# hmomin/FinEnvs

Hardware: NVIDIA B200
Metric: env_steps_per_sec (higher is better)
Workload: dtype f32/f64

## Files before the change

finenvs_b200/csrc/fe_step.cu:

```cuda
#include "finenvs_b200.h"
#include "fe_common.cuh"
#include "fe_metrics.cuh"

#include <cuda.h>
#include <cuda_runtime.h>
#include <stdint.h>
#include <stdlib.h>

#include <atomic>
#include <mutex>
#include <vector>

namespace {

constexpr int kThreads = 128;
constexpr int kMaxTileEnvs = kThreads;
constexpr int kSmemHeader = 16;
constexpr int kSmemMax = 226 * 1024;

__device__ __forceinline__ float fmul(float a, float b) { return __fmul_rn(a, b); }
__device__ __forceinline__ float fadd(float a, float b) { return __fadd_rn(a, b); }
__device__ __forceinline__ float fsub(float a, float b) { return __fsub_rn(a, b); }
__device__ __forceinline__ double dmul(double a, double b) { return __dmul_rn(a, b); }
__device__ __forceinline__ double dadd(double a, double b) { return __dadd_rn(a, b); }
// ... 423 lines not shown
    }
    __syncthreads();

    if (warp < kPipeBook) {
        const bool ahead = !kObserve && k.rewards_mirror != nullptr;
        auto tile_env = [&](int t) { return ((int64_t)blockIdx.x + (int64_t)t * gridDim.x) * TE + lane; };
        auto tile_active = [&](int t) { return t < ntiles && lane < TE && tile_env(t) < p.num_envs; };
        EnvLoads ld, ld_next;
        ld.seg = 0; ld.ptr = 0; ld.cash = 0.0f; ld.lng = 0.0f; ld.sht = 0.0f; ld.act = 0.0f; ld.margin = 0.0;
        ld_next = ld;
        if (ahead && tile_active(warp)) ld = env_load_state(st, actions, tile_env(warp));
        for (int t = warp; t < ntiles; t += kPipeBook) {
            const int q = t % kPipeQ;
            if (ahead && tile_active(t + kPipeBook)) ld_next = env_load_state(st, actions, tile_env(t + kPipeBook));
            mbar_wait(desc_free(q), ((t / kPipeQ) & 1) ^ 1);
            const int64_t env0 = ((int64_t)blockIdx.x + (int64_t)t * gridDim.x) * TE;
            const int nvalid = (int)min((int64_t)TE, p.num_envs - env0);
            EnvResult r;
            r.done = 0; r.newly_terminated = 0; r.fin_return = 0.0; r.fin_len = 0; r.row0 = 0; r.posfeat = 0.0;
            const bool active = lane < nvalid;
            if (active) {
                const int64_t i = env0 + lane;
                if (kObserve) r = env_observe(p, s, st, k, i);
                else {
                    if (!ahead) ld = env_load_state(st, actions, i);
                    r = env_compute<OutT>(p, s, st, k, i, ld, env_load_bar(p, s, ld), rewards, dones, stats != nullptr, step);
                }
                d_row0[q * TE + lane] = r.row0;
                reinterpret_cast<OutT *>(d_pf + q * TE)[lane] = (OutT)r.posfeat;
            }
            ld = ld_next;
            if (!kObserve && k.dones_bits_out) {
                const unsigned word = __ballot_sync(0xFFFFFFFFu, active && r.done);
                if (lane == 0) k.dones_bits_out[env0 >> 5] = word;
            }
            if (!kObserve) accumulate_stats(stats, r, active);
            __syncwarp();
            if (lane == 0) mbar_arrive(desc_full(q));
        }
    } else {
        const int mtid = tid - kPipeBook * 32;
        int e_u[RPT], j_u[RPT];
#pragma unroll
        for (int u = 0; u < RPT; ++u) {
            e_u[u] = (mtid + u * kMovers) / W;
            j_u[u] = (mtid + u * kMovers) - e_u[u] * W;
        }
        const Row4<OutT> *series_rows = reinterpret_cast<const Row4<OutT> *>(s.logret);
        auto tile_rows = [&](int t) {
            const int64_t env0 = ((int64_t)blockIdx.x + (int64_t)t * gridDim.x) * TE;
            return (int)min((int64_t)TE, p.num_envs - env0) * W;
        };
        auto gather = [&](int t, Row4<OutT>(&buf)[RPT]) {
            const int q = t % kPipeQ;
            mbar_wait(desc_full(q), (t / kPipeQ) & 1);
            const int nrows = tile_rows(t);
            const uint32_t stage = kPipeSIn > 0 ? smem_u32(in_ring + (t % (kPipeSIn > 0 ? kPipeSIn : 1)) * in_stage) : 0u;
#pragma unroll
            for (int u = 0; u < RPT; ++u) {
                const int r = mtid + u * kMovers;
                if (r < nrows) {
                    const Row4<OutT> *src = series_rows + d_row0[q * TE + e_u[u]] + j_u[u];
                    if constexpr (kPipeSIn == 0) {
                        buf[u] = ldg_row(src);
                    } else {
                        cp_async16(stage + (uint32_t)r * sizeof(Row4<OutT>), src);
                        if constexpr (sizeof(OutT) == 8)
                            cp_async16(stage + (uint32_t)r * sizeof(Row4<OutT>) + 16, reinterpret_cast<const char *>(src) + 16);
                    }
                }
            }
            if constexpr (kPipeSIn > 0) cp_async_arrive_noinc(in_full(t % (kPipeSIn > 0 ? kPipeSIn : 1)));
        };
        Row4<OutT> cur[RPT], nxt[RPT];
        constexpr int kAhead = kPipeSIn > 0 ? kPipeSIn : 1;
        if constexpr (kPipeSIn == 0) {
            if (ntiles > 0) gather(0, cur);
        } else {
            for (int t = 0; t < kAhead && t < ntiles; ++t) gather(t, nxt);
        }
        for (int t = 0; t < ntiles; ++t) {
            const int q = t % kPipeQ, so = t % kPipeSOut;
            const int64_t env0 = ((int64_t)blockIdx.x + (int64_t)t * gridDim.x) * TE;
            const int nrows = tile_rows(t);
            if constexpr (kPipeSIn == 0) {
                if (t + 1 < ntiles) gather(t + 1, nxt);
            } else {
                mbar_wait(in_full(t % kAhead), (t / kAhead) & 1);
                const Row4<OutT> *in_rows = reinterpret_cast<const Row4<OutT> *>(in_ring + (t % kAhead) * in_stage);
#pragma unroll
                for (int u = 0; u < RPT; ++u) {
                    const int r = mtid + u * kMovers;
                    if (r < nrows) cur[u] = in_rows[r];
                }
            }
            if (t >= kPipeSOut) {
                if (mtid == 0) asm volatile("cp.async.bulk.wait_group.read %0;" ::"n"(kPipeSOut - 1) : "memory");
                named_bar_sync(1, kMovers);
            }
            OutT *out_tile = reinterpret_cast<OutT *>(out_ring + so * out_stage);
            const OutT *pf = reinterpret_cast<const OutT *>(d_pf + q * TE);
#pragma unroll
            for (int u = 0; u < RPT; ++u) {
                const int r = mtid + u * kMovers;
                if (r < nrows) {
                    OutT *o = out_tile + (size_t)r * 5;
                    if constexpr (sizeof(OutT) == 4) {
                        o[0] = cur[u].v.x; o[1] = cur[u].v.y; o[2] = cur[u].v.z; o[3] = cur[u].v.w;
                    } else {
                        o[0] = cur[u].a.x; o[1] = cur[u].a.y; o[2] = cur[u].b.x; o[3] = cur[u].b.y;
                    }
                    o[4] = pf[e_u[u]];
                }
            }
            const size_t out_bytes = (size_t)nrows * 5 * sizeof(OutT);
            OutT *dst = obs + (size_t)env0 * W * 5;
            if ((out_bytes & 15) == 0) {
                fence_proxy_async_smem();
                named_bar_sync(1, kMovers);
                if (mtid == 0) {
                    bulk_store_hint(dst, smem_u32(out_tile), (uint32_t)out_bytes, l2_policy_evict_first());
                    bulk_commit();
                }
            } else {
                named_bar_sync(1, kMovers);
                for (int f = mtid; f < nrows * 5; f += kMovers) dst[f] = out_tile[f];
                named_bar_sync(1, kMovers);
            }
            if constexpr (kPipeSIn == 0) {
                if (mtid == 0) mbar_arrive(desc_free(q));
#pragma unroll
                for (int u = 0; u < RPT; ++u) cur[u] = nxt[u];
            } else {
                if (mtid == 0) mbar_arrive(desc_free(q));
                if (t + kAhead < ntiles) gather(t + kAhead, nxt);
            }
        }
        if (mtid == 0) bulk_wait_read_all();
    }
}

#ifndef FE_GATHER_BOOK
#define FE_GATHER_BOOK 6
#endif
#ifndef FE_GATHER_MOVE
#define FE_GATHER_MOVE 12
#endif
#ifndef FE_GATHER_STAGES
#define FE_GATHER_STAGES 3
#endif
#ifndef FE_GATHER_FLUSH_SPINS
#define FE_GATHER_FLUSH_SPINS 2000
#endif
constexpr int kGaBook = FE_GATHER_BOOK;
constexpr int kGaMove = FE_GATHER_MOVE;
constexpr int kGaThreads = (kGaBook + kGaMove) * 32;
constexpr int kGaQ = 32;
constexpr int kGaMaxStages = 4;
constexpr int kGaBarBytes = 1280;
constexpr int kGaPitch = 80;

static_assert((2 * kGaQ + kGaMove * kGaMaxStages) * 8 + 16 <= kGaBarBytes, "mbarrier area too small");
__host__ __device__ inline int ga_row_bytes(bool f64) { return f64 ? 40 : 20; }
__host__ __device__ inline int ga_phase_shift(bool f64) { return f64 ? 1 : 2; }
__host__ __device__ inline int64_t ga_rows_per_phase(int64_t num_rows, int W, bool f64) {
    const int P = 1 << ga_phase_shift(f64);
    return (num_rows + P - 1) / P + (W + P - 1) / P + 8;
}
__host__ __device__ inline size_t ga_table_bytes(int64_t num_rows, int W, bool f64) {
    return (size_t)(1 << ga_phase_shift(f64)) * (size_t)ga_rows_per_phase(num_rows, W, f64) * kGaPitch + 4096;
}
__host__ __device__ inline int ga_parts(int W, bool f64) {
    const int wb = ga_row_bytes(f64) * W;
    if (W <= 0 || (wb % 16) != 0) return 0;
    if (wb <= 2048) return 1;
    if (wb <= 4096 && ((wb / 2) % kGaPitch) == 0 && W <= 128) return 2;
    return 0;
}
__host__ __device__ inline bool ga_window_ok(int W, bool f64) { return ga_parts(W, f64) != 0; }
__host__ __device__ inline uint32_t ga_slot_pitch(int W, bool f64) {
    const int parts = ga_parts(W, f64);
    return ((4u / (uint32_t)(parts ? parts : 1)) * ga_row_bytes(f64) * W + 127u) & ~127u;
}
template <typename OutT> __host__ __device__ inline size_t gather_desc_bytes() {
    return ((size_t)kGaQ * (4 + 32 * (4 + sizeof(OutT))) + 127) & ~(size_t)127;
}
template <typename OutT> __host__ __device__ inline size_t gather_smem_bytes(int W, int S) {
    return kGaBarBytes + gather_desc_bytes<OutT>() + (size_t)kGaMove * S * ga_slot_pitch(W, sizeof(OutT) == 8);
}

__device__ __forceinline__ void tma_gather4(uint32_t dst_smem, const CUtensorMap *map, int r0, int r1, int r2, int r3, uint32_t bar,
                                            uint64_t policy) {
    asm volatile(
        "cp.async.bulk.tensor.2d.shared::cluster.global.tile::gather4.mbarrier::complete_tx::bytes.L2::cache_hint"
        " [%0], [%1, {%2, %3, %4, %5, %6}], [%7], %8;"
        ::"r"(dst_smem), "l"(map), "r"(0), "r"(r0), "r"(r1), "r"(r2), "r"(r3), "r"(bar), "l"(policy)
        : "memory");
}

#ifdef FE_GATHER_CLOCKS
__device__ unsigned long long fe_gather_clk[16];
__device__ unsigned long long fe_gather_block_ns[3 * 160];
__device__ __forceinline__ unsigned long long ga_globaltimer() {
    unsigned long long t;
    asm volatile("mov.u64 %0, %%globaltimer;" : "=l"(t));
    return t;
}
#define GA_CLK(var) const long long var = clock64()
#define GA_ACC(slot, a, b) acc[slot] += (b) - (a)
#else
#define GA_CLK(var)
#define GA_ACC(slot, a, b)
#endif

template <typename OutT, bool kObserve, int kParts>
__global__ void __launch_bounds__(kGaThreads, 1)
fe_gather_kernel(const __grid_constant__ CUtensorMap tmap, const FeParams p, const FeSeries s, const FeState st, const Consts k,
                 const float *__restrict__ actions, OutT *__restrict__ obs, OutT *__restrict__ rewards,
                 int32_t *__restrict__ dones, FeStats *stats, const uint64_t step_arg, const uint64_t *__restrict__ step_dev,
                 const int S, const int rows_per_phase, unsigned int *__restrict__ sched) {
    constexpr bool kF64 = sizeof(OutT) == 8;
    constexpr int kUnitEnvs = 4 / kParts;
    constexpr int kTileUnits = 32 / kUnitEnvs;
    constexpr int kUnitShift = kParts == 1 ? 3 : 4;
    static_assert(kParts == 1 || kParts == 2, "a window is fetched in one or two parts");
    extern __shared__ __align__(128) unsigned char smem[];
    const uint64_t step = step_dev ? *step_dev : step_arg;
    const int W = p.window;
    const int tid = threadIdx.x, warp = tid >> 5, lane = tid & 31;
    const int ntiles_all = (int)((p.num_envs + 31) / 32);
    const uint32_t bars = smem_u32(smem);
    auto desc_full = [&](int q) { return bars + 8u * q; };
    auto desc_free = [&](int q) { return bars + 8u * (kGaQ + q); };
    auto slot_full = [&](int m, int si) { return bars + 8u * (2 * kGaQ + m * kGaMaxStages + si); };
    unsigned int *claim = reinterpret_cast<unsigned int *>(smem + kGaBarBytes - 16);
    int32_t *d_tile = reinterpret_cast<int32_t *>(smem + kGaBarBytes);
    int32_t *d_row = d_tile + kGaQ;
    OutT *d_pf = reinterpret_cast<OutT *>(smem + kGaBarBytes + (size_t)kGaQ * (4 + 32 * 4));
    unsigned char *ring = smem + kGaBarBytes + gather_desc_bytes<OutT>();
    const uint32_t pitch = ga_slot_pitch(W, kF64);

#ifdef FE_GATHER_CLOCKS
    if (tid == 0 && blockIdx.x < 160) {
        unsigned smid;
        asm volatile("mov.u32 %0, %%smid;" : "=r"(smid));
        fe_gather_block_ns[3 * blockIdx.x] = ga_globaltimer();
        fe_gather_block_ns[3 * blockIdx.x + 2] = smid;
        fe_gather_block_ns[3 * blockIdx.x + 1] = 0;
    }
#endif
    if (tid == 0) {
        for (int q = 0; q < kGaQ; ++q) { mbar_init(desc_full(q), 1); mbar_init(desc_free(q), kTileUnits); }
        for (int m = 0; m < kGaMove; ++m)
            for (int si = 0; si < kGaMaxStages; ++si) mbar_init(slot_full(m, si), 1);
        claim[0] = 0; claim[1] = 0;
        mbar_fence_init();
    }
    __syncthreads();

    if (warp < kGaBook) {
        const int shift = ga_phase_shift(kF64);
#ifdef FE_GATHER_CLOCKS
        long long acc[16] = {0};
        int ntl = 0;
#endif
        const bool ahead = !kObserve && k.rewards_mirror != nullptr;
        auto take_claim = [&](int &n, int &t) {
            n = 0; t = 0;
            if (lane == 0) {
                while (atomicCAS(&claim[0], 0u, 1u) != 0u) {}
                n = (int)claim[1];
                claim[1] = (unsigned)n + 1;
                t = (int)atomicAdd(&sched[0], 1u);
                __threadfence_block();
                atomicExch(&claim[0], 0u);
            }
            n = __shfl_sync(0xFFFFFFFFu, n, 0);
            t = __shfl_sync(0xFFFFFFFFu, t, 0);
        };
        auto first_hop = [&](int t, EnvLoads &ld) {
            const int64_t i = (int64_t)t * 32 + lane;
            if (!kObserve && t < ntiles_all && i < p.num_envs) ld = env_load_state(st, actions, i);
        };
        int n, t, n_next = 0, t_next = 0;
        EnvLoads ld, ld_next;
        ld.seg = 0; ld.ptr = 0; ld.cash = 0.0f; ld.lng = 0.0f; ld.sht = 0.0f; ld.act = 0.0f; ld.margin = 0.0;
        ld_next = ld;
        take_claim(n, t);
        first_hop(t, ld);
        for (;;) {
            const int q = n & (kGaQ - 1);
            if (ahead && t < ntiles_all) {
                take_claim(n_next, t_next);
                first_hop(t_next, ld_next);
            }
            GA_CLK(c0);
            if (lane == 0) mbar_wait(desc_free(q), ((n / kGaQ) & 1) ^ 1);
            __syncwarp();
            GA_CLK(c1);
            GA_ACC(8, c0, c1);
            if (t >= ntiles_all) {
                if (lane == 0) { d_tile[q] = -1; mbar_arrive(desc_full(q)); }
                break;
            }
            const int64_t i = (int64_t)t * 32 + lane;
            const bool active = i < p.num_envs;
            EnvResult r;
            r.done = 0; r.newly_terminated = 0; r.fin_return = 0.0; r.fin_len = 0; r.row0 = 0; r.posfeat = 0.0;
            if (active) {
                if (kObserve) r = env_observe(p, s, st, k, i);
                else r = env_compute<OutT>(p, s, st, k, i, ld, env_load_bar(p, s, ld), rewards, dones, stats != nullptr, step);
            }
            d_row[q * 32 + lane] = (int32_t)((r.row0 & ((1 << shift) - 1)) * rows_per_phase + (r.row0 >> shift));
            d_pf[q * 32 + lane] = (OutT)r.posfeat;
            if (lane == 0) d_tile[q] = t;
            if (!kObserve && k.dones_bits_out) {
                const unsigned word = __ballot_sync(0xFFFFFFFFu, active && r.done);
                if (lane == 0) k.dones_bits_out[t] = word;
            }
            if (!kObserve) accumulate_stats(stats, r, active);
            __syncwarp();
            if (lane == 0) mbar_arrive(desc_full(q));
            GA_CLK(c2);
            GA_ACC(9, c1, c2);
#ifdef FE_GATHER_CLOCKS
            ++ntl;
#endif
            if (ahead) { n = n_next; t = t_next; ld = ld_next; }
            else { take_claim(n, t); first_hop(t, ld); }
        }
        if (!kObserve && k.dones_bits_host) {
            if (lane == 0) {
                __threadfence();
                atomicAdd(&sched[2], 1u);
            }
            if (warp == 0) {
                int ok = 1;
                if (lane == 0) {
                    const unsigned want = gridDim.x * (unsigned)kGaBook;
                    int spins = 0;
                    while (ld_acquire_gpu(&sched[2]) < want) {
                        if (++spins > FE_GATHER_FLUSH_SPINS) { ok = 0; break; }
                        __nanosleep(100);
                    }
                    if (!ok) atomicOr(&sched[3], 1u);
                }
                ok = __shfl_sync(0xFFFFFFFFu, ok, 0);
                const int per = (((ntiles_all + (int)gridDim.x - 1) / (int)gridDim.x) + 31) & ~31;
                const int w_begin = (int)blockIdx.x * per;
                const int w_end = !ok ? w_begin : w_begin + per < ntiles_all ? w_begin + per : ntiles_all;
                constexpr int kBatch = 8;
                for (int w0 = w_begin + lane; w0 < w_end; w0 += kBatch * 32) {
                    uint32_t v[kBatch];
#pragma unroll
                    for (int j = 0; j < kBatch; ++j) v[j] = w0 + 32 * j < w_end ? __ldcg(k.dones_bits_out + w0 + 32 * j) : 0u;
#pragma unroll
                    for (int j = 0; j < kBatch; ++j)
                        if (w0 + 32 * j < w_end) k.dones_bits_host[w0 + 32 * j] = v[j];
                }
            }
        }
#ifdef FE_GATHER_CLOCKS
        if (blockIdx.x == 0 && tid == 0) { fe_gather_clk[8] = acc[8]; fe_gather_clk[9] = acc[9]; fe_gather_clk[10] = ntl; }
#endif
    } else {
#ifdef FE_GATHER_CLOCKS
        long long acc[16] = {0};
        const long long mover_t0 = clock64();
#endif
        const int m = warp - kGaBook;
        const uint32_t row_b = (uint32_t)ga_row_bytes(kF64) * W, unit_b = kUnitEnvs * row_b;
        const int part_rows = (int)(row_b / 2) / kGaPitch;
        unsigned char *slots = ring + (size_t)m * S * pitch;
        constexpr int kRounds = (kParts == 1 && kF64) ? 2 : 4;
        uint32_t round_mask = 0;
#pragma unroll
        for (int kk = 0; kk < kRounds; ++kk) round_mask |= (uint32_t)(lane + 32 * kk < W) << kk;
        const uint32_t env_stride = (uint32_t)W * 5;
        const uint64_t keep = l2_policy_evict_last(), stream_out = l2_policy_evict_first();
        static_assert((kGaQ & (kGaQ - 1)) == 0, "kGaQ must be a power of two");
        int iss_u = m, iss_si = 0;
        int issued = 0;
        bool open = true;
        auto issue = [&]() {
            const int n = iss_u >> kUnitShift, g = iss_u & (kTileUnits - 1), q = n & (kGaQ - 1);
            GA_CLK(c0);
            mbar_wait(desc_full(q), (n / kGaQ) & 1);
            GA_CLK(c1);
            GA_ACC(4, c0, c1);
            if (d_tile[q] < 0) { open = false; return; }
            int4 rows4;
            if constexpr (kParts == 1) {
                rows4 = *reinterpret_cast<const int4 *>(d_row + q * 32 + 4 * g);
            } else {
                const int2 r2 = *reinterpret_cast<const int2 *>(d_row + q * 32 + 2 * g);
                rows4 = make_int4(r2.x, r2.x + part_rows, r2.y, r2.y + part_rows);
            }
#ifdef FE_GATHER_NOLOAD
            if (rows4.x == -12345)
#endif
            {
                mbar_arrive_expect_tx(slot_full(m, iss_si), unit_b);
                tma_gather4(smem_u32(slots + (size_t)iss_si * pitch), &tmap, rows4.x, rows4.y, rows4.z, rows4.w, slot_full(m, iss_si),
                            keep);
            }
#ifdef FE_GATHER_NOLOAD
            mbar_arrive(slot_full(m, iss_si));
#endif
            ++issued;
            iss_u += kGaMove;
            iss_si = iss_si + 1 == S ? 0 : iss_si + 1;
            GA_CLK(c2);
            GA_ACC(5, c1, c2);
        };
        if (lane == 0)
            for (int i = 0; i < S && open; ++i) issue();
        int u = m, si = 0;
        uint32_t slot_phase = 0;
        int n_iss = __shfl_sync(0xFFFFFFFFu, issued, 0);
        for (int i = 0; i < n_iss; ++i) {
            const int n = u >> kUnitShift, g = u & (kTileUnits - 1), q = n & (kGaQ - 1);
            GA_CLK(c0);
            if (lane == 0) mbar_wait(slot_full(m, si), (slot_phase >> si) & 1u);
            __syncwarp();
            GA_CLK(c1);
            GA_ACC(0, c0, c1);
            unsigned char *slot = slots + (size_t)si * pitch;
            const OutT *pf = d_pf + q * 32 + kUnitEnvs * g;
            OutT *col = reinterpret_cast<OutT *>(slot) + 5 * lane + 4;
#ifdef FE_GATHER_NOPF
            if (pf[0] == (OutT)12345.678)
#endif
#pragma unroll
            for (int e = 0; e < kUnitEnvs; ++e) {
                const OutT v = pf[e];
#pragma unroll
                for (int kk = 0; kk < kRounds; ++kk)
                    if (round_mask & (1u << kk)) col[e * env_stride + 160 * kk] = v;
            }
            GA_CLK(c1b);
            GA_ACC(1, c1, c1b);
#ifndef FE_GATHER_NOFENCE
            fence_proxy_async_smem();
#endif
            __syncwarp();
            GA_CLK(c2);
            GA_ACC(11, c1b, c2);
            if (lane == 0) {
                const int64_t env0 = (int64_t)d_tile[q] * 32 + kUnitEnvs * g;
                const int64_t left = p.num_envs - env0;
                const int nv = left >= kUnitEnvs ? kUnitEnvs : (left > 0 ? (int)left : 0);
#ifdef FE_GATHER_NOSTORE
                if (nv > 4)
#else
                if (nv > 0)
#endif
                {
                    bulk_store_hint(obs + (size_t)env0 * W * 5, smem_u32(slot), (uint32_t)nv * row_b, stream_out);
                    bulk_commit();
                }
                mbar_arrive(desc_free(q));
                GA_CLK(c3);
                GA_ACC(2, c2, c3);
                if (open) {
                    bulk_wait_read_all();
                    GA_CLK(c4);
                    GA_ACC(3, c3, c4);
                    issue();
                }
            }
            __syncwarp();
            n_iss = __shfl_sync(0xFFFFFFFFu, issued, 0);
            slot_phase ^= 1u << si;
            u += kGaMove;
            si = si + 1 == S ? 0 : si + 1;
        }
        if (lane == 0) bulk_wait_read_all();
#ifdef FE_GATHER_CLOCKS
        if (lane == 0 && blockIdx.x < 160) atomicMax(&fe_gather_block_ns[3 * blockIdx.x + 1], ga_globaltimer());
        if (blockIdx.x == 0 && m == 0 && lane == 0) { for (int c = 0; c < 6; ++c) fe_gather_clk[c] = acc[c]; fe_gather_clk[6] = issued; fe_gather_clk[11] = acc[11]; fe_gather_clk[12] = 0; fe_gather_clk[13] = clock64() - mover_t0; }
#endif
    }
    __syncthreads();
    if (tid == 0) {
        __threadfence();
        unsigned send_all = 0;
        if (atomicAdd(&sched[1], 1u) == gridDim.x - 1) {
            __threadfence();
            send_all = ld_acquire_gpu(&sched[3]);
            sched[0] = 0;
            sched[1] = 0;
            sched[2] = 0;
            sched[3] = 0;
            __threadfence();
        }
        claim[2] = send_all;
    }
    if (!kObserve && k.dones_bits_host) {
        __syncthreads();
        if (claim[2])
            for (int w = tid; w < ntiles_all; w += kGaThreads) k.dones_bits_host[w] = __ldcg(k.dones_bits_out + w);
    }
}

template <typename OutT>
__global__ void __launch_bounds__(256)
fe_obs_table_kernel(const OutT *__restrict__ logret, const int64_t num_rows, const int64_t rows_per_phase,
                    unsigned char *__restrict__ table) {
    constexpr bool kF64 = sizeof(OutT) == 8;
    const int shift = ga_phase_shift(kF64);
    const int64_t idx = (int64_t)blockIdx.x * blockDim.x + threadIdx.x;
    const int64_t r = idx >> shift;
    const int kk = (int)(idx & ((1 << shift) - 1));
    if (r >= num_rows || r < kk) return;
    OutT *dst = reinterpret_cast<OutT *>(table + (size_t)kk * kGaPitch * rows_per_phase + (size_t)(r - kk) * ga_row_bytes(kF64));
    const OutT *src = logret + r * 4;
    dst[0] = src[0]; dst[1] = src[1]; dst[2] = src[2]; dst[3] = src[3];
    dst[4] = (OutT)0;
}

template <typename OutT, bool kObserve>
__global__ void __launch_bounds__(kThreads)
fe_direct_kernel(const FeParams p, const FeSeries s, const FeState st, const Consts k, const float *__restrict__ actions,
                 OutT *__restrict__ obs, OutT *__restrict__ rewards, int32_t *__restrict__ dones, FeStats *stats,
                 const uint64_t step_arg, const uint64_t *__restrict__ step_dev) {
    __shared__ int64_t sh_row0[kThreads];
    const uint64_t step = step_dev ? *step_dev : step_arg;
    __shared__ OutT sh_pf[kThreads];
    const int W = p.window;
    const int tid = threadIdx.x;
    const int64_t env0 = (int64_t)blockIdx.x * kThreads;
    const int nvalid = (int)min((int64_t)kThreads, p.num_envs - env0);
    const bool active = tid < nvalid;
    EnvResult r;
    r.done = 0; r.newly_terminated = 0; r.fin_return = 0.0; r.fin_len = 0; r.row0 = 0; r.posfeat = 0.0;
    if (active) {
        const int64_t i = env0 + tid;
        if (kObserve) r = env_observe(p, s, st, k, i);
        else r = env_step<OutT>(p, s, st, k, i, actions, rewards, dones, stats != nullptr, step);
    }
    sh_row0[tid] = r.row0;
    sh_pf[tid] = (OutT)r.posfeat;
    if (!kObserve) accumulate_stats(stats, r, active);
    __syncthreads();
    const int lane = tid & 31, warp = tid >> 5;
    const OutT *lr = reinterpret_cast<const OutT *>(s.logret);
    const int nvals = W * 5;
    for (int e = warp; e < nvalid; e += kThreads / 32) {
        const OutT *src = lr + sh_row0[e] * 4;
        OutT *dst = obs + (size_t)(env0 + e) * nvals;
        const OutT pfe = sh_pf[e];
        for (int f = lane; f < nvals; f += 32) {
            const int j = f / 5, c = f - j * 5;
            dst[f] = c == 4 ? pfe : __ldg(src + j * 4 + c);
        }
    }
}

template <typename OutT, bool kObserve>
__global__ void __launch_bounds__(kThreads)
fe_lazy_kernel(const FeParams p, const FeSeries s, const FeState st, const Consts k, const float *__restrict__ actions,
               int64_t *__restrict__ row0_out, OutT *__restrict__ pf_out, OutT *__restrict__ rewards,
               int32_t *__restrict__ dones, FeStats *stats, const uint64_t step_arg, const uint64_t *__restrict__ step_dev) {
    const uint64_t step = step_dev ? *step_dev : step_arg;
    const int64_t i = (int64_t)blockIdx.x * kThreads + threadIdx.x;
    const bool active = i < p.num_envs;
    EnvResult r;
    r.done = 0; r.newly_terminated = 0; r.fin_return = 0.0; r.fin_len = 0; r.row0 = 0; r.posfeat = 0.0;
    if (active) {
        if (kObserve) r = env_observe(p, s, st, k, i);
        else r = env_step<OutT>(p, s, st, k, i, actions, rewards, dones, stats != nullptr, step);
        row0_out[i] = r.row0;
        pf_out[i] = (OutT)r.posfeat;
    }
    if (!kObserve) accumulate_stats(stats, r, active);
}

template <typename OutT>
__global__ void __launch_bounds__(kThreads)
fe_materialize_kernel(const int64_t N, const int W, const OutT *__restrict__ logret, const int64_t *__restrict__ row0,
                      const OutT *__restrict__ pf, const int64_t *__restrict__ index, OutT *__restrict__ obs) {
    const int lane = threadIdx.x & 31;
    const int64_t e = ((int64_t)blockIdx.x * kThreads + threadIdx.x) >> 5;
    if (e >= N) return;
    const int64_t h = index ? index[e] : e;
    const OutT *src = logret + row0[h] * 4;
    OutT *dst = obs + (size_t)e * W * 5;
    const OutT pfe = pf[h];
    for (int f = lane; f < W * 5; f += 32) {
        const int j = f / 5, c = f - j * 5;
        dst[f] = c == 4 ? pfe : __ldg(src + j * 4 + c);
    }
}

constexpr int kGoMaxWarps = 16;
constexpr int kGoBarBytes = kGoMaxWarps * kGaMaxStages * 8;

template <typename OutT, int kParts>
__global__ void __launch_bounds__(kGoMaxWarps * 32)
fe_gather_obs_kernel(const __grid_constant__ CUtensorMap tmap, const int64_t count, const int W, const int64_t *__restrict__ row0,
                     const OutT *__restrict__ pf, const int64_t *__restrict__ index, OutT *__restrict__ obs, const int S,
                     const int rows_per_phase) {
    constexpr bool kF64 = sizeof(OutT) == 8;
    constexpr int kUnitEnvs = 4 / kParts;
    constexpr int kTileUnits = 32 / kUnitEnvs;
    constexpr int kRounds = (kParts == 1 && kF64) ? 2 : 4;
    static_assert(kParts == 1 || kParts == 2, "a window is fetched in one or two parts");
    extern __shared__ __align__(128) unsigned char smem[];
    const int warp = threadIdx.x >> 5, lane = threadIdx.x & 31, nwarps = blockDim.x >> 5;
    const uint32_t pitch = ga_slot_pitch(W, kF64);
    const uint32_t bars = smem_u32(smem) + 8u * (uint32_t)(warp * S);
    unsigned char *slots = smem + kGoBarBytes + (size_t)warp * S * pitch;
    const uint32_t row_b = (uint32_t)ga_row_bytes(kF64) * W, unit_b = kUnitEnvs * row_b;
    const int part_rows = (int)(row_b / 2) / kGaPitch;
    const int shift = ga_phase_shift(kF64);
    const int64_t gw = (int64_t)blockIdx.x * nwarps + warp, NW = (int64_t)gridDim.x * nwarps;
    const int64_t ntiles = (count + 31) / 32;
    if (gw >= ntiles) return;
    const int64_t my_tiles = (ntiles - gw + NW - 1) / NW;
    const int64_t last_tile = gw + (my_tiles - 1) * NW;
    const int last_units = (int)(((count - last_tile * 32 < 32 ? count - last_tile * 32 : 32) + kUnitEnvs - 1) / kUnitEnvs);
    const int64_t n_units = (my_tiles - 1) * kTileUnits + last_units;

    if (lane == 0) {
        for (int si = 0; si < S; ++si) mbar_init(bars + 8u * si, 1);
        mbar_fence_init();
    }
    __syncwarp();

    auto load = [&](int64_t k, int &row, OutT &v) {
        int64_t b = (gw + k * NW) * 32 + lane;
        if (b >= count) b = count - 1;
// ... 554 lines not shown
    StepKernel kern;
    int te;
    int sin;
    int S;
    int threads;
};
StepChoice choose_kernel(const FeParams &p, bool gather_ready, bool f64, int sms) {
    StepChoice c = {K_DIRECT, 0, 0, 0, kThreads};
    if (p.num_assets > 1 || p.variant == FE_VARIANT_PORTFOLIO) { c.kern = K_PORTFOLIO; return c; }
    if (p.variant == FE_VARIANT_SPLIT) { c.kern = K_SPLIT; return c; }
    const bool worth_persistent = p.num_envs >= (int64_t)4 * sms * 32;
    if (p.variant == FE_VARIANT_GATHER || p.variant == FE_VARIANT_AUTO) {
        c.S = pick_gather_stages(p.window, f64);
        if (p.variant == FE_VARIANT_GATHER) {
            c.kern = !gather_ready ? K_ERR_TABLE : c.S == 0 ? K_ERR_SMEM : K_GATHER;
            return c;
        }
        const bool no_gather = env_override("FE_NO_GATHER") != 0;
        if (!no_gather && gather_ready && c.S > 0 && worth_persistent && p.window >= 24 && gather_table_resident(p, f64)) {
            c.kern = K_GATHER;
            return c;
        }
    }
    if (p.variant == FE_VARIANT_PIPE || p.variant == FE_VARIANT_AUTO) {
        const int ov_sin = env_override("FE_PIPE_FLAVOUR");
        c.sin = ov_sin == 1 ? 0 : ov_sin == 2 ? kPipeSInStream : pick_pipe_stages(p, f64);
        c.te = pick_pipe_envs(p.window, f64, c.sin);
        if (c.te == 0 && p.variant == FE_VARIANT_PIPE) { c.kern = K_ERR_SMEM; return c; }
        if (c.te > 0 && (p.variant == FE_VARIANT_PIPE || (worth_persistent && p.window >= 24))) { c.kern = K_PIPE; return c; }
        if (c.te == 0 && p.variant == FE_VARIANT_AUTO) { c.kern = K_SPLIT; return c; }
    }
    c.te = p.variant == FE_VARIANT_DIRECT ? 0 : pick_tile_envs(p.window, f64, &c.threads);
    if (p.variant == FE_VARIANT_TILE && c.te == 0) { c.kern = K_ERR_SMEM; return c; }
    if (c.te > 0) {
        const int ov_e = env_override("FE_TILE_ENVS"), ov_t = env_override("FE_TILE_THREADS");
        const size_t sz = f64 ? 8 : 4;
        if (ov_e >= 4 && kSmemHeader + 16 + (size_t)(ov_e & ~3) * (p.window * 9 * sz + sz) <= (size_t)kSmemMax) c.te = ov_e & ~3;
        if (ov_t >= 32 && ov_t <= kThreads) c.threads = ov_t & ~31;
        if (c.te > c.threads) c.te = c.threads;
        c.kern = K_TILE;
    }
    return c;
}

template <typename Kern> int opt_in_smem(Kern kern, std::atomic<uint32_t> &done_mask, int device) {
    const uint32_t bit = 1u << (device & 15);
    if (done_mask.load(std::memory_order_acquire) & bit) return 0;
    cudaError_t e = cudaFuncSetAttribute(kern, cudaFuncAttributeMaxDynamicSharedMemorySize, (int)kSmemMax);
    if (e != cudaSuccess) return (int)e;
    done_mask.fetch_or(bit, std::memory_order_release);
    return 0;
}

typedef CUresult (*EncodeTiledFn)(CUtensorMap *, CUtensorMapDataType, cuuint32_t, void *, const cuuint64_t *, const cuuint64_t *,
                                  const cuuint32_t *, const cuuint32_t *, CUtensorMapInterleave, CUtensorMapSwizzle,
                                  CUtensorMapL2promotion, CUtensorMapFloatOOBfill);
struct TmapEntry {
    const void *base;
    int64_t rows;
    int inner_bytes, device;
    CUtensorMap map;
};
int gather_tensor_map(const void *table, int64_t total_rows, int inner_bytes, int device, CUtensorMap *out) {
    static std::mutex mu;
    static std::vector<TmapEntry> cache;
    static EncodeTiledFn encode = nullptr;
    std::lock_guard<std::mutex> lock(mu);
    for (const TmapEntry &e : cache)
        if (e.base == table && e.rows == total_rows && e.inner_bytes == inner_bytes && e.device == device) { *out = e.map; return 0; }
    if (!encode) {
        void *fn = nullptr;
        cudaDriverEntryPointQueryResult q;
        cudaError_t e = cudaGetDriverEntryPoint("cuTensorMapEncodeTiled", &fn, cudaEnableDefault, &q);
        if (e != cudaSuccess) return (int)e;
        if (!fn || q != cudaDriverEntryPointSuccess) return FE_EDRIVER;
        encode = (EncodeTiledFn)fn;
    }
    TmapEntry n;
    n.base = table; n.rows = total_rows; n.inner_bytes = inner_bytes; n.device = device;
    const cuuint64_t dims[2] = {(cuuint64_t)(inner_bytes / 8), (cuuint64_t)total_rows};
    const cuuint64_t strides[1] = {(cuuint64_t)kGaPitch};
    const cuuint32_t box[2] = {(cuuint32_t)(inner_bytes / 8), 1}, elem_strides[2] = {1, 1};
    const CUresult r = encode(&n.map, CU_TENSOR_MAP_DATA_TYPE_UINT64, 2, const_cast<void *>(table), dims, strides, box, elem_strides,
                              CU_TENSOR_MAP_INTERLEAVE_NONE, CU_TENSOR_MAP_SWIZZLE_NONE, CU_TENSOR_MAP_L2_PROMOTION_NONE,
                              CU_TENSOR_MAP_FLOAT_OOB_FILL_NONE);
    if (r != CUDA_SUCCESS) return FE_EDRIVER;
    if (cache.size() >= 64) cache.erase(cache.begin());
    cache.push_back(n);
    *out = n.map;
    return 0;
}

template <typename OutT, bool kObserve>
int launch(const FeParams &p, const FeSeries &s, const FeState &st, const float *actions, void *obs, void *rewards,
           int32_t *dones, FeStats *stats, uint64_t step, cudaStream_t stream, const uint64_t *step_dev = nullptr,
           void *rewards_mirror = nullptr, int32_t *dones_mirror = nullptr, uint32_t *dones_bits_mirror = nullptr,
           uint32_t *dones_bits_stage = nullptr, int *packed_inline = nullptr) {
    Consts k = make_consts(p);
    k.rewards_mirror = rewards_mirror;
    k.dones_mirror = dones_mirror;
    int sms = 0;
    int rc = device_sm_count(p.device, &sms);
    if (rc) return rc;
    const StepChoice c = choose_kernel(p, s.obs_table && st.sched, sizeof(OutT) == 8, sms);
    const bool inline_pack = dones_bits_mirror && dones_bits_stage && (c.kern == K_GATHER || (c.kern == K_PIPE && c.te == 32));
    const int pack_mode = env_override("FE_PACK_MODE");
    if (inline_pack) {
        k.dones_bits_out = pack_mode == 1 ? dones_bits_mirror : dones_bits_stage;
        if (c.kern == K_GATHER && pack_mode == 0) k.dones_bits_host = dones_bits_mirror;
    }
    if (packed_inline) *packed_inline = !inline_pack ? 0 : (pack_mode == 1 || (c.kern == K_GATHER && pack_mode == 0)) ? 1 : 2;
    switch (c.kern) {
    case K_ERR_SMEM: return FE_ESMEM;
    case K_ERR_TABLE: return FE_EINVAL;
    case K_PORTFOLIO: {
        if ((uintptr_t)obs & 15) return FE_EALIGN;
        const int P = p.window * p.num_assets;
        int CH = 512;
        const int ov_ch = env_override("FE_PORT_CHUNK");
        if (ov_ch >= 4) CH = ov_ch & ~3;
        if (CH > ((P + 3) & ~3)) CH = (P + 3) & ~3;
        const size_t smem = port_smem_bytes<OutT>(CH);
        if (smem > (size_t)kSmemMax) return FE_ESMEM;
        auto skern = fe_portfolio_stream_kernel<OutT>;
        static std::atomic<uint32_t> configured{0};
        if ((rc = opt_in_smem(skern, configured, p.device))) return rc;
        fe_portfolio_book_kernel<OutT, kObserve><<<(unsigned)((p.num_envs + kBookWarps - 1) / kBookWarps), kBookWarps * 32, 0, stream>>>(
            p, s, st, k, actions, (OutT *)obs, (OutT *)rewards, dones, stats, step, step_dev);
        skern<<<(unsigned)p.num_envs, kPortThreads, smem, stream>>>(p, s, (OutT *)obs, CH);
        break;
    }
    case K_SPLIT: {
        if ((uintptr_t)obs & 7) return FE_EALIGN;
        fe_book_kernel<OutT, kObserve><<<(unsigned)((p.num_envs + kThreads - 1) / kThreads), kThreads, 0, stream>>>(
            p, s, st, k, actions, (OutT *)obs, (OutT *)rewards, dones, stats, step, step_dev);
        const int ov_b = env_override("FE_STREAM_BLOCKS_PER_SM");
        int64_t blocks = (int64_t)sms * (ov_b > 0 ? ov_b : 6);
        const int64_t need = (p.num_envs * 32 + kStreamThreads - 1) / kStreamThreads;
        if (blocks > need) blocks = need;
        fe_stream_kernel<OutT><<<(unsigned)blocks, kStreamThreads, 0, stream>>>(p.num_envs, p.window, (const OutT *)s.logret, (OutT *)obs);
        break;
    }
    case K_GATHER: {
        if ((uintptr_t)obs & 15) return FE_EALIGN;
        constexpr bool f64 = sizeof(OutT) == 8;
        const int64_t rpp = ga_rows_per_phase(p.num_rows, p.window, f64);
        const int64_t total_rows = rpp << ga_phase_shift(f64);
        if (total_rows >= ((int64_t)1 << 31)) return FE_EINVAL;
        const int parts = ga_parts(p.window, f64);
        CUtensorMap tmap;
        if ((rc = gather_tensor_map(s.obs_table, total_rows, ga_row_bytes(f64) * p.window / parts, p.device, &tmap))) return rc;
        const int64_t ntiles = (p.num_envs + 31) / 32;
        const unsigned blocks = (unsigned)(ntiles < sms ? ntiles : sms);
        const size_t smem = gather_smem_bytes<OutT>(p.window, c.S);
        if (parts == 1) {
            auto kern = fe_gather_kernel<OutT, kObserve, 1>;
            static std::atomic<uint32_t> configured{0};
            if ((rc = opt_in_smem(kern, configured, p.device))) return rc;
            kern<<<blocks, kGaThreads, smem, stream>>>(tmap, p, s, st, k, actions, (OutT *)obs, (OutT *)rewards, dones, stats, step,
                                                       step_dev, c.S, (int)rpp, st.sched);
        } else {
            auto kern = fe_gather_kernel<OutT, kObserve, 2>;
            static std::atomic<uint32_t> configured{0};
            if ((rc = opt_in_smem(kern, configured, p.device))) return rc;
            kern<<<blocks, kGaThreads, smem, stream>>>(tmap, p, s, st, k, actions, (OutT *)obs, (OutT *)rewards, dones, stats, step,
                                                       step_dev, c.S, (int)rpp, st.sched);
        }
        break;
    }
    case K_PIPE: {
        if ((uintptr_t)obs & 15) return FE_EALIGN;
        const int64_t ntiles = (p.num_envs + c.te - 1) / c.te;
        const unsigned blocks = (unsigned)(ntiles < sms ? ntiles : sms);
        if (c.sin == 0) {
            auto kern = fe_pipe_kernel<OutT, kObserve, 0>;
            static std::atomic<uint32_t> configured{0};
            if ((rc = opt_in_smem(kern, configured, p.device))) return rc;
            kern<<<blocks, kPipeThreads, pipe_smem_bytes<OutT>(c.te, p.window, c.sin), stream>>>(
                p, s, st, k, actions, (OutT *)obs, (OutT *)rewards, dones, stats, step, step_dev, c.te);
        } else {
            auto kern = fe_pipe_kernel<OutT, kObserve, kPipeSInStream>;
            static std::atomic<uint32_t> configured{0};
            if ((rc = opt_in_smem(kern, configured, p.device))) return rc;
            kern<<<blocks, kPipeThreads, pipe_smem_bytes<OutT>(c.te, p.window, c.sin), stream>>>(
                p, s, st, k, actions, (OutT *)obs, (OutT *)rewards, dones, stats, step, step_dev, c.te);
        }
        break;
    }
    case K_TILE: {
        if ((uintptr_t)obs & 15) return FE_EALIGN;
        const size_t smem = tile_smem_bytes<OutT>(c.te, p.window);
        auto kern = fe_tile_kernel<OutT, kObserve>;
        static std::atomic<uint32_t> configured{0};
        if ((rc = opt_in_smem(kern, configured, p.device))) return rc;
        const int64_t blocks = (p.num_envs + c.te - 1) / c.te;
        kern<<<(unsigned)blocks, c.threads, smem, stream>>>(p, s, st, k, actions, (OutT *)obs, (OutT *)rewards, dones,
                                                             stats, step, step_dev, c.te);
        break;
    }
    case K_DIRECT: {
        const int64_t blocks = (p.num_envs + kThreads - 1) / kThreads;
        fe_direct_kernel<OutT, kObserve><<<(unsigned)blocks, kThreads, 0, stream>>>(
            p, s, st, k, actions, (OutT *)obs, (OutT *)rewards, dones, stats, step, step_dev);
        break;
    }
    }
    return (int)cudaGetLastError();
}

enum ObsPath { OBS_NONE, OBS_TMA, OBS_LSU };
ObsPath choose_obs_path(const FeParams &p, const FeSeries &s) {
    if (p.num_assets != 1) return OBS_NONE;
    const bool f64 = p.out_f64 != 0;
    return s.obs_table && ga_parts(p.window, f64) > 0 && gather_table_resident(p, f64) ? OBS_TMA : OBS_LSU;
}

template <typename OutT>
int gather_obs(const FeParams &p, const FeSeries &s, const int64_t *row0, const void *pf, const int64_t *index, int64_t count,
               void *obs, cudaStream_t stream) {
    constexpr bool f64 = sizeof(OutT) == 8;
    if (choose_obs_path(p, s) != OBS_TMA || (((uintptr_t)obs | (uintptr_t)s.obs_table) & 15)) {
        const int64_t blocks = (count * 32 + kThreads - 1) / kThreads;
        fe_materialize_kernel<OutT><<<(unsigned)blocks, kThreads, 0, stream>>>(count, p.window, (const OutT *)s.logret, row0,
                                                                               (const OutT *)pf, index, (OutT *)obs);
        return (int)cudaGetLastError();
    }
    int sms = 0;
    int rc = device_sm_count(p.device, &sms);
    if (rc) return rc;
    const int64_t rpp = ga_rows_per_phase(p.num_rows, p.window, f64);
    const int parts = ga_parts(p.window, f64);
    CUtensorMap tmap;
    if ((rc = gather_tensor_map(s.obs_table, rpp << ga_phase_shift(f64), ga_row_bytes(f64) * p.window / parts, p.device, &tmap)))
        return rc;
    const size_t pitch = ga_slot_pitch(p.window, f64), room = (size_t)kSmemMax - kGoBarBytes;
    int S = 3;
    if (room / (S * pitch) < 8) S = 2;
    const int warps = (int)(room / (S * pitch) < (size_t)kGoMaxWarps ? room / (S * pitch) : kGoMaxWarps);
    const size_t smem = kGoBarBytes + (size_t)warps * S * pitch;
    int per_sm = (int)((size_t)(228 * 1024) / (smem + 1024));
    per_sm = per_sm < 1 ? 1 : per_sm > 4 ? 4 : per_sm;
    const int64_t need = ((count + 31) / 32 + warps - 1) / warps;
    const unsigned blocks = (unsigned)(need < (int64_t)sms * per_sm ? need : (int64_t)sms * per_sm);
    if (parts == 1) {
        auto kern = fe_gather_obs_kernel<OutT, 1>;
        static std::atomic<uint32_t> configured{0};
        if ((rc = opt_in_smem(kern, configured, p.device))) return rc;
        kern<<<blocks, warps * 32, smem, stream>>>(tmap, count, p.window, row0, (const OutT *)pf, index, (OutT *)obs, S, (int)rpp);
    } else {
        auto kern = fe_gather_obs_kernel<OutT, 2>;
        static std::atomic<uint32_t> configured{0};
        if ((rc = opt_in_smem(kern, configured, p.device))) return rc;
        kern<<<blocks, warps * 32, smem, stream>>>(tmap, count, p.window, row0, (const OutT *)pf, index, (OutT *)obs, S, (int)rpp);
    }
    return (int)cudaGetLastError();
}

__global__ void fe_bump_kernel(uint64_t *counter) { *counter += 1; }

constexpr int kBtThreads = 256;
constexpr int kBtWarps = kBtThreads / 32;

struct BacktestEnvIO {
    int32_t seg, ptr;
    float cash, lng, sht;
    double margin;
    int term;
    float eret;
    int32_t elen;
    double rew;
    int done;
    __device__ __forceinline__ void set_seg(int32_t v) { seg = v; }
    __device__ __forceinline__ int terminated() const { return term; }
    __device__ __forceinline__ void set_terminated() { term = 1; }
    __device__ __forceinline__ float ep_return() const { return eret; }
    __device__ __forceinline__ void set_ep_return(float v) { eret = v; }
    __device__ __forceinline__ int32_t ep_len() const { return elen; }
    __device__ __forceinline__ void set_ep_len(int32_t v) { elen = v; }
    __device__ __forceinline__ void finish(int32_t ptr_, float cash_, float lng_, float sht_, double margin_, double rew_,
                                           int done_) {
        ptr = ptr_; cash = cash_; lng = lng_; sht = sht_; margin = margin_; rew = rew_; done = done_;
    }
};

template <typename T, typename Op>
__device__ __forceinline__ T bt_block_reduce(T v, Op op, T *sh) {
#pragma unroll
    for (int o = 16; o > 0; o >>= 1) v = op(v, __shfl_xor_sync(0xFFFFFFFFu, v, o));
    __syncthreads();
    if ((threadIdx.x & 31) == 0) sh[threadIdx.x >> 5] = v;
    __syncthreads();
    if (threadIdx.x == 0)
        for (int w = 1; w < kBtWarps; ++w) v = op(v, sh[w]);
    return v;
}

struct TradeRule {
    __device__ __forceinline__ void load(int32_t) {}
    __device__ __forceinline__ float action(float v, const BacktestEnvIO &, const EpisodeRun &) const { return v; }
};
struct TargetRule {
    const double *__restrict__ exits;
    float ms, scale;
    double stop, take;
    __device__ __forceinline__ void load(int32_t c) {
        if (exits) { stop = __ldg(exits + 2 * (int64_t)c); take = __ldg(exits + 2 * (int64_t)c + 1); }
    }
    __device__ __forceinline__ float action(float v, const BacktestEnvIO &e, const EpisodeRun &run) const {
        float T = rintf(fmul(v, scale));
        T = T < -ms ? -ms : (T > ms ? ms : T);
        if (exits && (dsub(run.peak, run.sum) >= stop || run.sum >= take)) T = 0.0f;
        return __fdiv_rn(fsub(T, fsub(e.lng, e.sht)), scale);
    }
};

template <typename OutT, typename Rule>
__device__ __forceinline__ void
backtest_run(const FeParams p, const FeSeries s, const FeState st, const Consts k, const FeMetricsState m,
             const int64_t capacity, FeStats *stats, const float *__restrict__ signal, const int32_t *__restrict__ column,
// ... 436 lines not shown
}

const char *fe_gather_obs_kernel_name(const FeParams *p, const FeSeries *s) {
    if (!p || !s) return "";
    const bool f64 = p->out_f64 != 0;
    switch (choose_obs_path(*p, *s)) {
    case OBS_TMA: return f64 ? "fe_gather_obs_kernel<double>" : "fe_gather_obs_kernel<float>";
    case OBS_LSU: return f64 ? "fe_materialize_kernel<double>" : "fe_materialize_kernel<float>";
    default: return "none (handles exist for single-asset series only)";
    }
}

static int step_host_impl(const FeParams *p, const FeSeries *s, const FeState *st, const float *actions_host, float *actions_dev,
                          void *obs_dev, void *rewards_dev, int32_t *dones_dev, void *rewards_host, int32_t *dones_host,
                          uint32_t *dones_bits_host, FeStats *stats_dev, uint64_t step_counter, void *stream) {
    if (!p || !s || !st || !actions_host || !actions_dev || !rewards_host || (!dones_host == !dones_bits_host)) return FE_EINVAL;
    int rc = check_common(p, s, st);
    if (rc) return rc;
    if (!obs_dev || !rewards_dev || !dones_dev) return FE_EINVAL;
    if (stats_dev && !p->evaluate && (!st->ep_return || !st->ep_len)) return FE_EINVAL;
    DeviceGuard guard(p->device);
    if (guard.rc) return guard.rc;
    cudaStream_t q = (cudaStream_t)stream;
    const int64_t n = p->num_envs;
    const int A = p->num_assets;
    const size_t osz = p->out_f64 ? 8 : 4;
    const void *dones_any = dones_host ? (const void *)dones_host : (const void *)dones_bits_host;
    int sms = 0;
    if ((rc = device_sm_count(p->device, &sms))) return rc;
    if (!env_override("FE_HOST_NO_ZEROCOPY")) {
        cudaPointerAttributes aa, ar, ad;
        const bool ok = cudaPointerGetAttributes(&aa, actions_host) == cudaSuccess && aa.type == cudaMemoryTypeHost &&
                        aa.devicePointer && cudaPointerGetAttributes(&ar, rewards_host) == cudaSuccess &&
                        ar.type == cudaMemoryTypeHost && ar.devicePointer &&
                        cudaPointerGetAttributes(&ad, dones_any) == cudaSuccess && ad.type == cudaMemoryTypeHost &&
                        ad.devicePointer;
        (void)cudaGetLastError();
        const StepKernel kk = choose_kernel(*p, s->obs_table && st->sched, p->out_f64 != 0, sms).kern;
        const bool small = n <= 32768;
        if (ok && ((kk != K_TILE && kk != K_DIRECT) || small)) {
            const float *a = (const float *)aa.devicePointer;
            int32_t *dmirror = dones_host ? (int32_t *)ad.devicePointer : nullptr;
            uint32_t *bmirror = dones_bits_host ? (uint32_t *)ad.devicePointer : nullptr;
            uint32_t *stage = reinterpret_cast<uint32_t *>(actions_dev);
            int packed_inline = 0;
            rc = p->out_f64 ? launch<double, false>(*p, *s, *st, a, obs_dev, rewards_dev, dones_dev, stats_dev, step_counter, q,
                                                    nullptr, ar.devicePointer, dmirror, bmirror, stage, &packed_inline)
                            : launch<float, false>(*p, *s, *st, a, obs_dev, rewards_dev, dones_dev, stats_dev, step_counter, q,
                                                   nullptr, ar.devicePointer, dmirror, bmirror, stage, &packed_inline);
            if (rc) return rc;
            if (dones_bits_host && packed_inline != 1) {
                const int64_t nwords = (n + 31) / 32;
                if (packed_inline == 0 && small) {
                    fe_pack_dones_kernel<<<(unsigned)((n + 255) / 256), 256, 0, q>>>(dones_dev, n, (uint32_t *)ad.devicePointer);
                } else {
                    if (packed_inline == 0)
                        fe_pack_dones_kernel<<<(unsigned)((n + 255) / 256), 256, 0, q>>>(dones_dev, n, stage);
                    fe_flush_bits_kernel<<<(unsigned)((nwords + 255) / 256), 256, 0, q>>>(stage, nwords, (uint32_t *)ad.devicePointer);
                }
                if ((rc = (int)cudaGetLastError())) return rc;
            }
            return (int)cudaStreamSynchronize(q);
        }
    }
    const int ov_chunks = env_override("FE_HOST_CHUNKS");
    int chunks = ov_chunks > 0 ? ov_chunks : 4;
    int64_t per = ((n + chunks - 1) / chunks + 1023) & ~(int64_t)1023;
    if (per < 16384) per = 16384;
    chunks = (int)((n + per - 1) / per);
    HostPipe *hp = nullptr;
    if (chunks > 1) {
        hp = host_pipe(p->device);
        if (!hp) return (int)cudaGetLastError();
        cudaError_t e = cudaEventRecord(hp->start, q);
        if (e != cudaSuccess) return (int)e;
    }
    for (int c = 0; c < chunks; ++c) {
        const int64_t off = (int64_t)c * per, cnt = off + per <= n ? per : n - off;
        cudaStream_t cs = hp ? hp->s[c % kHostStreams] : q;
        cudaError_t e;
        if (hp && c < kHostStreams && (e = cudaStreamWaitEvent(cs, hp->start, 0)) != cudaSuccess) return (int)e;
        e = cudaMemcpyAsync(actions_dev + off * A, actions_host + off * A, (size_t)cnt * A * sizeof(float),
                            cudaMemcpyHostToDevice, cs);
        if (e != cudaSuccess) return (int)e;
        FeParams pc = *p;
        pc.num_envs = cnt;
        pc.env_id_base = p->env_id_base + off;
        if (pc.variant == FE_VARIANT_GATHER) pc.variant = FE_VARIANT_AUTO;
        FeState sc = *st;
        sc.sched = nullptr;
        sc.seg += off; sc.ptr += off; sc.cash += off;
        sc.long_sh += off * A; sc.short_sh += off * A; sc.margin += off * A;
        if (sc.terminated) sc.terminated += off;
        if (sc.ep_return) sc.ep_return += off;
        if (sc.ep_len) sc.ep_len += off;
        const size_t obs_off = (size_t)off * p->window * 5 * A * osz;
        rc = p->out_f64 ? launch<double, false>(pc, *s, sc, actions_dev + off * A, (char *)obs_dev + obs_off, (char *)rewards_dev + off * osz,
                                                dones_dev + off, stats_dev, step_counter, cs)
                        : launch<float, false>(pc, *s, sc, actions_dev + off * A, (char *)obs_dev + obs_off, (char *)rewards_dev + off * osz,
                                               dones_dev + off, stats_dev, step_counter, cs);
        if (rc) return rc;
        e = cudaMemcpyAsync((char *)rewards_host + off * osz, (char *)rewards_dev + off * osz, (size_t)cnt * osz,
                            cudaMemcpyDeviceToHost, cs);
        if (e != cudaSuccess) return (int)e;
        if (dones_host) {
            e = cudaMemcpyAsync(dones_host + off, dones_dev + off, (size_t)cnt * sizeof(int32_t), cudaMemcpyDeviceToHost, cs);
        } else {
            uint32_t *bits_dev = reinterpret_cast<uint32_t *>(actions_dev + off * A);
            fe_pack_dones_kernel<<<(unsigned)((cnt + 255) / 256), 256, 0, cs>>>(dones_dev + off, cnt, bits_dev);
            if ((rc = (int)cudaGetLastError())) return rc;
            e = cudaMemcpyAsync(dones_bits_host + (off >> 5), bits_dev, (size_t)((cnt + 31) / 32) * 4, cudaMemcpyDeviceToHost, cs);
        }
        if (e != cudaSuccess) return (int)e;
    }
    if (hp) {
        for (int k = 0; k < kHostStreams && k < chunks; ++k) {
            cudaError_t e = cudaEventRecord(hp->done[k], hp->s[k]);
            if (e != cudaSuccess) return (int)e;
            if ((e = cudaStreamWaitEvent(q, hp->done[k], 0)) != cudaSuccess) return (int)e;
        }
    }
    return (int)cudaStreamSynchronize(q);
}

int fe_step_host(const FeParams *p, const FeSeries *s, const FeState *st, const float *actions_host, float *actions_dev,
                 void *obs_dev, void *rewards_dev, int32_t *dones_dev, void *rewards_host, int32_t *dones_host,
                 FeStats *stats_dev, uint64_t step_counter, void *stream) {
    if (!dones_host) return FE_EINVAL;
    return step_host_impl(p, s, st, actions_host, actions_dev, obs_dev, rewards_dev, dones_dev, rewards_host, dones_host, nullptr,
                          stats_dev, step_counter, stream);
}

int fe_step_host_packed(const FeParams *p, const FeSeries *s, const FeState *st, const float *actions_host, float *actions_dev,
                        void *obs_dev, void *rewards_dev, int32_t *dones_dev, void *rewards_host, uint32_t *dones_bits_host,
                        FeStats *stats_dev, uint64_t step_counter, void *stream) {
    if (!dones_bits_host) return FE_EINVAL;
    return step_host_impl(p, s, st, actions_host, actions_dev, obs_dev, rewards_dev, dones_dev, rewards_host, nullptr, dones_bits_host,
                          stats_dev, step_counter, stream);
}

int fe_reset_all(const FeParams *p, const FeSeries *s, const FeState *st, uint64_t step_counter, int32_t redraw,
                 void *stream) {
    int rc = check_common(p, s, st);
    if (rc) return rc;
    DeviceGuard guard(p->device);
    if (guard.rc) return guard.rc;
    fe_reset_all_kernel<<<(unsigned)((p->num_envs + 255) / 256), 256, 0, (cudaStream_t)stream>>>(*p, *s, *st, step_counter,
                                                                                                 redraw);
    return (int)cudaGetLastError();
}

#ifdef FE_GATHER_CLOCKS
int fe_debug_gather_clocks(unsigned long long out[16]) { return (int)cudaMemcpyFromSymbol(out, fe_gather_clk, 128); }
int fe_debug_gather_blocks(unsigned long long out[480]) { return (int)cudaMemcpyFromSymbol(out, fe_gather_block_ns, 480 * 8); }
#endif

void fe_philox(uint64_t seed, uint64_t env_id, uint64_t step, uint32_t kind, uint32_t out[4]) {
    philox4x32_10(seed, env_id, step, kind, out);
}

}
```

Before: 4.686 billion.

## Overlap gather kernel prologue with prior launch via PDL and pre-assign first tiles

Launches the gather kernel with programmatic dependent launch, so its mbarrier setup and tensormap prefetch can run while the previous kernel finishes. It waits on griddepcontrol before reading the step counter, and signals dependents once tile claiming ends. Each bookkeeping warp also gets a statically assigned first tile, which skips the initial atomic claim and starts state loads earlier. The risks are a subtle dependency-ordering bug if any global reads happen before the wait, and a scheduler offset change that must stay consistent with the reset of the sched counter.

```diff
diff --git a/finenvs_b200/csrc/fe_step.cu b/finenvs_b200/csrc/fe_step.cu
--- a/finenvs_b200/csrc/fe_step.cu
+++ b/finenvs_b200/csrc/fe_step.cu
@@ -599,6 +599,12 @@
 #ifndef FE_GATHER_FLUSH_SPINS
 #define FE_GATHER_FLUSH_SPINS 2000
 #endif
+#ifndef FE_GATHER_WARM
+#define FE_GATHER_WARM 1
+#endif
+#ifndef FE_GATHER_PDL
+#define FE_GATHER_PDL 1
+#endif
 constexpr int kGaBook = FE_GATHER_BOOK;
 constexpr int kGaMove = FE_GATHER_MOVE;
 constexpr int kGaThreads = (kGaBook + kGaMove) * 32;
@@ -647,7 +653,7 @@
 
 #ifdef FE_GATHER_CLOCKS
 __device__ unsigned long long fe_gather_clk[16];
-__device__ unsigned long long fe_gather_block_ns[3 * 160];
+__device__ unsigned long long fe_gather_block_ns[4 * 160];
 __device__ __forceinline__ unsigned long long ga_globaltimer() {
     unsigned long long t;
     asm volatile("mov.u64 %0, %%globaltimer;" : "=l"(t));
@@ -672,7 +678,6 @@
     constexpr int kUnitShift = kParts == 1 ? 3 : 4;
     static_assert(kParts == 1 || kParts == 2, "a window is fetched in one or two parts");
     extern __shared__ __align__(128) unsigned char smem[];
-    const uint64_t step = step_dev ? *step_dev : step_arg;
     const int W = p.window;
     const int tid = threadIdx.x, warp = tid >> 5, lane = tid & 31;
     const int ntiles_all = (int)((p.num_envs + 31) / 32);
@@ -687,21 +692,38 @@
     unsigned char *ring = smem + kGaBarBytes + gather_desc_bytes<OutT>();
     const uint32_t pitch = ga_slot_pitch(W, kF64);
 
+    if (tid == 0) {
+        asm volatile("prefetch.tensormap [%0];" ::"l"(reinterpret_cast<uint64_t>(&tmap)) : "memory");
+        for (int q = 0; q < kGaQ; ++q) { mbar_init(desc_full(q), 1); mbar_init(desc_free(q), kTileUnits); }
+        for (int m = 0; m < kGaMove; ++m)
+            for (int si = 0; si < kGaMaxStages; ++si) mbar_init(slot_full(m, si), 1);
+        claim[0] = 0; claim[1] = FE_GATHER_WARM ? kGaBook : 0;
+        mbar_fence_init();
+    }
+    asm volatile("griddepcontrol.wait;" ::: "memory");
+    const uint64_t step = step_dev ? *step_dev : step_arg;
 #ifdef FE_GATHER_CLOCKS
     if (tid == 0 && blockIdx.x < 160) {
         unsigned smid;
         asm volatile("mov.u32 %0, %%smid;" : "=r"(smid));
-        fe_gather_block_ns[3 * blockIdx.x] = ga_globaltimer();
-        fe_gather_block_ns[3 * blockIdx.x + 2] = smid;
-        fe_gather_block_ns[3 * blockIdx.x + 1] = 0;
+        fe_gather_block_ns[4 * blockIdx.x] = ga_globaltimer();
+        fe_gather_block_ns[4 * blockIdx.x + 2] = smid;
+        fe_gather_block_ns[4 * blockIdx.x + 1] = 0;
+        fe_gather_block_ns[4 * blockIdx.x + 3] = ~0ull;
     }
 #endif
-    if (tid == 0) {
-        for (int q = 0; q < kGaQ; ++q) { mbar_init(desc_full(q), 1); mbar_init(desc_free(q), kTileUnits); }
-        for (int m = 0; m < kGaMove; ++m)
-            for (int si = 0; si < kGaMaxStages; ++si) mbar_init(slot_full(m, si), 1);
-        claim[0] = 0; claim[1] = 0;
-        mbar_fence_init();
+    const bool ahead = !kObserve && k.rewards_mirror != nullptr;
+    auto first_hop = [&](int t, EnvLoads &ld) {
+        const int64_t i = (int64_t)t * 32 + lane;
+        if (!kObserve && t < ntiles_all && i < p.num_envs) ld = env_load_state(st, actions, i);
+    };
+    int n = 0, t = 0;
+    EnvLoads ld;
+    ld.seg = 0; ld.ptr = 0; ld.cash = 0.0f; ld.lng = 0.0f; ld.sht = 0.0f; ld.act = 0.0f; ld.margin = 0.0;
+    if (FE_GATHER_WARM && warp < kGaBook) {
+        n = warp;
+        t = (int)blockIdx.x + (int)gridDim.x * warp;
+        first_hop(t, ld);
     }
     __syncthreads();
 
@@ -711,30 +733,26 @@
         long long acc[16] = {0};
         int ntl = 0;
 #endif
-        const bool ahead = !kObserve && k.rewards_mirror != nullptr;
+        const int claimed_base = FE_GATHER_WARM ? (int)gridDim.x * kGaBook : 0;
         auto take_claim = [&](int &n, int &t) {
             n = 0; t = 0;
             if (lane == 0) {
                 while (atomicCAS(&claim[0], 0u, 1u) != 0u) {}
                 n = (int)claim[1];
                 claim[1] = (unsigned)n + 1;
-                t = (int)atomicAdd(&sched[0], 1u);
+                t = claimed_base + (int)atomicAdd(&sched[0], 1u);
                 __threadfence_block();
                 atomicExch(&claim[0], 0u);
             }
             n = __shfl_sync(0xFFFFFFFFu, n, 0);
             t = __shfl_sync(0xFFFFFFFFu, t, 0);
         };
-        auto first_hop = [&](int t, EnvLoads &ld) {
-            const int64_t i = (int64_t)t * 32 + lane;
-            if (!kObserve && t < ntiles_all && i < p.num_envs) ld = env_load_state(st, actions, i);
-        };
-        int n, t, n_next = 0, t_next = 0;
-        EnvLoads ld, ld_next;
-        ld.seg = 0; ld.ptr = 0; ld.cash = 0.0f; ld.lng = 0.0f; ld.sht = 0.0f; ld.act = 0.0f; ld.margin = 0.0;
-        ld_next = ld;
-        take_claim(n, t);
-        first_hop(t, ld);
+        int n_next = 0, t_next = 0;
+        EnvLoads ld_next = ld;
+        if (!FE_GATHER_WARM) {
+            take_claim(n, t);
+            first_hop(t, ld);
+        }
         for (;;) {
             const int q = n & (kGaQ - 1);
             if (ahead && t < ntiles_all) {
@@ -776,6 +794,7 @@
             if (ahead) { n = n_next; t = t_next; ld = ld_next; }
             else { take_claim(n, t); first_hop(t, ld); }
         }
+        asm volatile("griddepcontrol.launch_dependents;" ::: "memory");
         if (!kObserve && k.dones_bits_host) {
             if (lane == 0) {
                 __threadfence();
@@ -903,6 +922,9 @@
                 if (nv > 0)
 #endif
                 {
+#ifdef FE_GATHER_CLOCKS
+                    if (i == 0 && blockIdx.x < 160) atomicMin(&fe_gather_block_ns[4 * blockIdx.x + 3], ga_globaltimer());
+#endif
                     bulk_store_hint(obs + (size_t)env0 * W * 5, smem_u32(slot), (uint32_t)nv * row_b, stream_out);
                     bulk_commit();
                 }
@@ -924,7 +946,7 @@
         }
         if (lane == 0) bulk_wait_read_all();
 #ifdef FE_GATHER_CLOCKS
-        if (lane == 0 && blockIdx.x < 160) atomicMax(&fe_gather_block_ns[3 * blockIdx.x + 1], ga_globaltimer());
+        if (lane == 0 && blockIdx.x < 160) atomicMax(&fe_gather_block_ns[4 * blockIdx.x + 1], ga_globaltimer());
         if (blockIdx.x == 0 && m == 0 && lane == 0) { for (int c = 0; c < 6; ++c) fe_gather_clk[c] = acc[c]; fe_gather_clk[6] = issued; fe_gather_clk[11] = acc[11]; fe_gather_clk[12] = 0; fe_gather_clk[13] = clock64() - mover_t0; }
 #endif
     }
@@ -1785,19 +1807,30 @@
         if ((rc = gather_tensor_map(s.obs_table, total_rows, ga_row_bytes(f64) * p.window / parts, p.device, &tmap))) return rc;
         const int64_t ntiles = (p.num_envs + 31) / 32;
         const unsigned blocks = (unsigned)(ntiles < sms ? ntiles : sms);
-        const size_t smem = gather_smem_bytes<OutT>(p.window, c.S);
+        cudaLaunchConfig_t cfg = {};
+        cfg.gridDim = dim3(blocks);
+        cfg.blockDim = dim3(kGaThreads);
+        cfg.dynamicSmemBytes = gather_smem_bytes<OutT>(p.window, c.S);
+        cfg.stream = stream;
+        cudaLaunchAttribute pdl[1];
+        pdl[0].id = cudaLaunchAttributeProgrammaticStreamSerialization;
+        pdl[0].val.programmaticStreamSerializationAllowed = 1;
+        cfg.attrs = pdl;
+        cfg.numAttrs = FE_GATHER_PDL ? 1 : 0;
         if (parts == 1) {
             auto kern = fe_gather_kernel<OutT, kObserve, 1>;
             static std::atomic<uint32_t> configured{0};
             if ((rc = opt_in_smem(kern, configured, p.device))) return rc;
-            kern<<<blocks, kGaThreads, smem, stream>>>(tmap, p, s, st, k, actions, (OutT *)obs, (OutT *)rewards, dones, stats, step,
-                                                       step_dev, c.S, (int)rpp, st.sched);
+            if ((rc = (int)cudaLaunchKernelEx(&cfg, kern, tmap, p, s, st, k, actions, (OutT *)obs, (OutT *)rewards, dones, stats, step,
+                                              step_dev, c.S, (int)rpp, st.sched)))
+                return rc;
         } else {
             auto kern = fe_gather_kernel<OutT, kObserve, 2>;
             static std::atomic<uint32_t> configured{0};
             if ((rc = opt_in_smem(kern, configured, p.device))) return rc;
-            kern<<<blocks, kGaThreads, smem, stream>>>(tmap, p, s, st, k, actions, (OutT *)obs, (OutT *)rewards, dones, stats, step,
-                                                       step_dev, c.S, (int)rpp, st.sched);
+            if ((rc = (int)cudaLaunchKernelEx(&cfg, kern, tmap, p, s, st, k, actions, (OutT *)obs, (OutT *)rewards, dones, stats, step,
+                                              step_dev, c.S, (int)rpp, st.sched)))
+                return rc;
         }
         break;
     }
@@ -2540,7 +2573,7 @@
 
 #ifdef FE_GATHER_CLOCKS
 int fe_debug_gather_clocks(unsigned long long out[16]) { return (int)cudaMemcpyFromSymbol(out, fe_gather_clk, 128); }
-int fe_debug_gather_blocks(unsigned long long out[480]) { return (int)cudaMemcpyFromSymbol(out, fe_gather_block_ns, 480 * 8); }
+int fe_debug_gather_blocks(unsigned long long out[640]) { return (int)cudaMemcpyFromSymbol(out, fe_gather_block_ns, 640 * 8); }
 #endif
 
 void fe_philox(uint64_t seed, uint64_t env_id, uint64_t step, uint32_t kind, uint32_t out[4]) {
```

Measured after the change: 4.742 billion, median of 6. +1.2%, better.
